# ictnlp/StreamSpeech

Measured on AMD Instinct MI355X. Metric: real-time factor (RTFx = audio seconds / wall seconds) + utterances/sec, offline S2ST fr-en, higher is better.
Workload: dtype f32

## Files before the change

### include/streamspeech_hip.h

```cpp
#ifndef STREAMSPEECH_HIP_H
#define STREAMSPEECH_HIP_H

#include <stddef.h>
#include <stdint.h>

#ifdef __cplusplus
extern "C" {
#endif

#define SS_ABI_VERSION 2

typedef struct ss_model ss_model;
typedef struct ss_vocoder ss_vocoder;
typedef struct ss_scratch ss_scratch;
typedef struct ss_stream_pool ss_stream_pool;

typedef struct ss_config {
  int32_t input_feat, conv_channels, conv_kernel;
  int32_t enc_dim, enc_ffn, enc_heads, enc_layers, dw_kernel;
  int32_t src_vocab, tgt_vocab;
  int32_t mt_layers, dec_dim, dec_ffn, dec_heads;
  int32_t t2u_layers, unit_layers, unit_vocab, ctc_upsample;
  int32_t pad, eos, unk;
  int32_t max_rel_pos;
// ... 418 lines not shown
int ss_debug_last_logits(ss_model* m, void* stream, float* d_out, int64_t cap_floats, int* h_rows, int* h_cols);

int ss_op_ffn_fused(void* stream, const float* dX, int ldx, float* dY, int ldy, const float* ln_g, const float* ln_b,
                    const float* dW1, const float* db1, const float* dW2, const float* db2, float alpha,
                    const float* ln2_g, const float* ln2_b, int M, int D, int F);
int ss_debug_ffn(int grid, int row_tiles_per_wave, int enable);
int ss_debug_rtlin(int grid, int enable);
int ss_debug_conv_c64(int enable);
int ss_debug_conv_c256_rows(int rows);
int ss_debug_conv_c32(int enable);
int ss_debug_conv_c16(int enable);
int64_t ss_debug_enc_step_launches(void);
int ss_op_ln_linear(void* stream, const float* dX, int ldx, const float* ln_g, const float* ln_b, const float* dW,
                    const float* dbias, const float* dR, int ldr, float* dC, int ldc, int M, int N, int K, int act, float alpha,
                    int glu);
int ss_op_ln_linear_ex(void* stream, const float* dX, int ldx, const float* ln_g, const float* ln_b, float* ln_out, const float* dW,
                       const float* dbias, const float* dR, int ldr, float* dC, int ldc, int M, int N, int K, int act, float alpha,
                       int glu, int canon);

int ss_debug_force_tile(int bm, int bn, int ks);
int ss_debug_sk_errors(void);
int ss_debug_attention_split(int v);
int ss_debug_attention_q16(int v);
int ss_debug_enc_step_inject_timeout(ss_model* m);
int ss_debug_scratch_audit(ss_scratch* sc, size_t* booked, size_t* held);
int ss_debug_mt_inject_timeout(ss_model* m);

int ss_op_conv_gemm(void* stream, const float* dA, int lda, const float* dW, const float* dbias,
                    const float* dR, int ldr, const float* dR2, int ldr2, float* dC, int ldc,
                    int M, int N, int Cin, int taps, int dil, int stride, int pad, int in_len,
                    int chunk, int in_act, float in_slope, int act, float alpha, float div, int glu);
typedef struct ss_op_conv_args {
  const float* A; const float* W; const float* bias; const float* R; const float* R2; float* C; float* C2;
  int32_t lda, ldc, ldr, ldr2, ldc2;
  int32_t M, N, Cin, taps, dil, stride, pad, in_len, chunk;
  int32_t in_act; float in_slope;
  int32_t act; float act_slope, alpha, div, c2_slope;
  int32_t glu;
  const int32_t* segs; int32_t nseg, max_seg_out;
  int32_t same_rows;
} ss_op_conv_args;
int ss_op_conv_gemm_ex(void* stream, const ss_op_conv_args* a);
int ss_op_conv_gemm_rows(void* stream, const ss_op_conv_args* a, int m_begin, const int32_t* seg_mb, const float* const* seg_A, int canon);
int ss_op_conv_pair(void* stream, const float* dA, int lda, const float* dW1, const float* db1, const float* dW2, const float* db2,
                    float* dC, int ldc, const float* dR2, int ldr2, float div, float* dC2, int ldc2, float c2_slope, int C, int taps,
                    int dil, int M, int in_len, float slope, const int32_t* d_segs, int nseg);
// ... 123 lines not shown
```

### streamspeech_amd/csrc/attention.hip

```cpp
#include "attn_tile.hpp"

#include <algorithm>
#include <cstdlib>

namespace ss {

void attention_debug_no_mfma(int v) { dispatch_edit([v](Dispatch& d) { d.attn_no_mfma = v; }); }
void attention_debug_q16(int v) { dispatch_edit([v](Dispatch& d) { d.attn_q16 = v; }); }
void attention_debug_split(int v) { dispatch_edit([v](Dispatch& d) { d.attn_split = v; }); }

constexpr int QB = 16;
constexpr int LDKS = DH + 1;

__device__ __forceinline__ float rdlane(float v, int l) {
  return __int_as_float(__builtin_amdgcn_readlane(__float_as_int(v), l));
}

template <bool RELPOS>
__global__ __launch_bounds__(256) void attention_kernel(AttnArgs p) {
  if (p.nseg > 0 && !seg_rebase(p, QB, RELPOS)) return;
  __shared__ float Ks[KT * LDKS];
  __shared__ float Vs[KT * DH];
  __shared__ float Ps[RELPOS ? (KT + QB - 1) * LDKS : 1];

  const int t = threadIdx.x, lane = t & 63, wave = t >> 6;
  const int h = blockIdx.y;
  const int i0 = blockIdx.x * QB;
  const int hoff = h * DH;
  const int qoff = p.Tk - p.Tq;
  const int q0 = p.q0;

  float qu[4], qv[4];
// ... 157 lines not shown
    const float corr = (m_run > -INFINITY) ? expf(m_run - mn) : 0.f;
    l_run = l_run * corr + wave_sum(pe);
    acc *= corr;
    m_run = mn;
#pragma unroll
    for (int u = 0; u < 64; ++u) acc = fmaf(rdlane(pe, u), vv[u], acc);
  }
  if (lane == 0) { part_m[wave] = m_run; part_l[wave] = l_run; }
  part_acc[wave][lane] = acc;
  __syncthreads();
  if (wave == 0) {
    float mt = fmaxf(fmaxf(part_m[0], part_m[1]), fmaxf(part_m[2], part_m[3]));
    float l = 0.f, o = 0.f;
#pragma unroll
    for (int w = 0; w < 4; ++w) {
      const float f = (part_m[w] > -INFINITY) ? expf(part_m[w] - mt) : 0.f;
      l += part_l[w] * f;
      o += part_acc[w][lane] * f;
    }
    p.O[(size_t)i * p.ldo + hoff + lane] = o / l;
  }
}

__global__ __launch_bounds__(256) void attention_mfma_kernel(AttnArgs p) {
  if (p.nseg > 0 && !seg_rebase(p, MQ, false)) return;
  __shared__ __attribute__((aligned(16))) float Ks[KT * LDT];
  __shared__ __attribute__((aligned(16))) float Vt[DH * LDT];
  const int t = threadIdx.x, lane = t & 63, wave = t >> 6;
  const int r = lane & 15, g = lane >> 4;
  const int h = blockIdx.y, hoff = h * DH;
  const int i0 = blockIdx.x * MQ;
  const int qoff = p.Tk - p.Tq;
  const int iq = i0 + wave * 16 + r;
  const bool q_ok = iq < p.Tq;

  f32x4 qf[4];
#pragma unroll
  for (int kk = 0; kk < 4; ++kk) {
    qf[kk] = f32x4{0.f, 0.f, 0.f, 0.f};
    if (q_ok) qf[kk] = *reinterpret_cast<const f32x4*>(p.Q + (size_t)iq * p.ldq + hoff + 16 * kk + 4 * g);
  }
  f32x4 o[4];
#pragma unroll
  for (int dt = 0; dt < 4; ++dt) o[dt] = f32x4{0.f, 0.f, 0.f, 0.f};
  float m_run = -INFINITY, l_run = 0.f;

  int kmax = p.Tk - p.k_mask_tail;
  const int ilast = min(i0 + MQ, p.Tq) - 1;
  if (p.causal) kmax = min(kmax, ilast + qoff + 1);
  if (p.chunk > 0) kmax = min(kmax, (ilast / p.chunk + 1) * p.chunk);
  int lim = p.Tk - p.k_mask_tail;
  if (p.causal) lim = min(lim, iq + qoff + 1);
  if (p.chunk > 0) lim = min(lim, (iq / p.chunk + 1) * p.chunk);
  if (!q_ok) lim = 0;

  for (int j0 = 0; j0 < kmax; j0 += KT) {
    __syncthreads();
    stage_kv_tile(Ks, Vt, p.K, p.V, p.ldk, p.ldv, p.Tk, j0, hoff, t);
    __syncthreads();

    f32x4 s[4];
#pragma unroll
    for (int kt = 0; kt < 4; ++kt) {
      s[kt] = f32x4{0.f, 0.f, 0.f, 0.f};
#pragma unroll
      for (int kk = 0; kk < 4; ++kk) {
        const f32x4 kf = *reinterpret_cast<const f32x4*>(Ks + (kt * 16 + r) * LDT + 16 * kk + 4 * g);
#pragma unroll
        for (int e = 0; e < 4; ++e) s[kt] = __builtin_amdgcn_mfma_f32_16x16x4f32(kf[e], qf[kk][e], s[kt], 0, 0, 0);
      }
    }
    const float corr = softmax_tile(s, j0, lim, p.scale, g, m_run, l_run);
    pv_tile(o, s, Vt, r, g, corr);
  }
  if (q_ok) store_rows(p.O, p.ldo, iq, hoff, g, o, l_run);
}

constexpr int PWIN = 2 * KT;
constexpr size_t kRelposLds = (size_t)(KT * LDT + DH * LDT + PWIN * LDT + 4 * 16 * LDG) * sizeof(float);

template <bool SPLIT>
__global__ __launch_bounds__(256) void attention_relpos_mfma_kernel(AttnArgs p) {
  if (!SPLIT && p.nseg > 0 && !seg_rebase(p, MQ, true)) return;
  extern __shared__ __attribute__((aligned(16))) float smem_rp[];
  float* Ks = smem_rp;
  float* Vt = Ks + KT * LDT;
  float* Ps = Vt + DH * LDT;
  const int t = threadIdx.x, lane = t & 63, wave = t >> 6;
  float* Gs = Ps + PWIN * LDT + wave * 16 * LDG;
  const int r = lane & 15, g = lane >> 4;
  const int h = blockIdx.y, hoff = h * DH;
  int qt = blockIdx.x, sp = 0;
  if (SPLIT) { const int nqt = gridDim.x / p.ksplit; sp = blockIdx.x / nqt; qt = blockIdx.x - sp * nqt; }
  const int i0 = qt * MQ;
  const int q0 = p.q0;
  const int iq = i0 + wave * 16 + r;
  const bool q_ok = iq < p.Tq;

  f32x4 quf[4], qvf[4];
  load_qu_qv(quf, qvf, p.Q, p.ldq, iq, q_ok, p.bias_u, p.bias_v, hoff, g);
  f32x4 o[4];
#pragma unroll
  for (int dt = 0; dt < 4; ++dt) o[dt] = f32x4{0.f, 0.f, 0.f, 0.f};
  float m_run = -INFINITY, l_run = 0.f;

  const int kmax = chunk_bound(p.Tk, p.chunk, min(i0 + MQ, p.Tq) - 1 + q0);
  const int lim = q_ok ? chunk_bound(p.Tk, p.chunk, iq + q0) : 0;
  int jbeg = 0, jend = kmax, s_eff = 1;
  if (SPLIT) {
    const int span = p.ktiles_per_split * KT;
    s_eff = (kmax + span - 1) / span;
    if (sp >= s_eff) return;
    jbeg = sp * span;
    jend = min(kmax, jbeg + span);
  }

  for (int j0 = jbeg; j0 < jend; j0 += KT) {
    __syncthreads();
    stage_kv_tile(Ks, Vt, p.K, p.V, p.ldk, p.ldv, p.Tk, j0, hoff, t);
    {
      const int pbase = j0 - (q0 + i0 + MQ - 1) + p.Tk - 1;
      for (int f = t; f < PWIN * (DH / 4); f += 256) {
        const int row = f >> 4, c4 = (f & 15) * 4;
        const int pr = pbase + row;
        f32x4 pv = {0.f, 0.f, 0.f, 0.f};
        if (row < PWIN - 1 && pr >= 0 && pr < 2 * p.Tk - 1)
          pv = *reinterpret_cast<const f32x4*>(p.P + (size_t)pr * p.ldp + hoff + c4);
        *reinterpret_cast<f32x4*>(Ps + row * LDT + c4) = pv;
      }
    }
    __syncthreads();

    f32x4 s[4];
#pragma unroll
    for (int kt = 0; kt < 4; ++kt) {
      s[kt] = f32x4{0.f, 0.f, 0.f, 0.f};
      f32x4 ga = {0.f, 0.f, 0.f, 0.f}, gb = {0.f, 0.f, 0.f, 0.f};
      const int lrow0 = 16 * (kt - wave) + (MQ - 16);
#pragma unroll
      for (int kk = 0; kk < 4; ++kk) {
        const f32x4 kf = *reinterpret_cast<const f32x4*>(Ks + (kt * 16 + r) * LDT + 16 * kk + 4 * g);
        const f32x4 pa = *reinterpret_cast<const f32x4*>(Ps + (lrow0 + r) * LDT + 16 * kk + 4 * g);
        const f32x4 pb = *reinterpret_cast<const f32x4*>(Ps + (lrow0 + 16 + r) * LDT + 16 * kk + 4 * g);
#pragma unroll
        for (int e = 0; e < 4; ++e) {
          s[kt] = __builtin_amdgcn_mfma_f32_16x16x4f32(kf[e], quf[kk][e], s[kt], 0, 0, 0);
          ga = __builtin_amdgcn_mfma_f32_16x16x4f32(pa[e], qvf[kk][e], ga, 0, 0, 0);
          gb = __builtin_amdgcn_mfma_f32_16x16x4f32(pb[e], qvf[kk][e], gb, 0, 0, 0);
        }
      }
      s[kt] += bd_skew(Gs, r, g, ga, gb);
    }
    const float corr = softmax_tile(s, j0, lim, p.scale, g, m_run, l_run);
    pv_tile(o, s, Vt, r, g, corr);
  }
  if (SPLIT && s_eff > 1) {
    using u32x4 = __attribute__((ext_vector_type(4))) unsigned;
    const int slot0 = (qt * (int)gridDim.y + h) * p.ksplit;
    {
      const __amdgpu_buffer_rsrc_t rs = __builtin_amdgcn_make_buffer_rsrc(
          (void*)(p.part + (size_t)(slot0 + sp) * ATTN_PART_FLOATS), 0, ATTN_PART_FLOATS * 4, 0x00020000);
#pragma unroll
      for (int dt = 0; dt < 4; ++dt) {
        u32x4 v;
#pragma unroll
        for (int e = 0; e < 4; ++e) v[e] = __float_as_uint(o[dt][e]);
        __builtin_amdgcn_raw_buffer_store_b128(v, rs, (dt * 256 + t) * 16, 0, 16);
      }
      const u32x4 ml = {__float_as_uint(m_run), __float_as_uint(l_run), 0u, 0u};
      __builtin_amdgcn_raw_buffer_store_b128(ml, rs, (4 * 256 + t) * 16, 0, 16);
    }
    __shared__ int s_last;
    unsigned* cnt = p.cnt + qt * (int)gridDim.y + h;
    if (!split_arrive(cnt, s_eff, &s_last)) return;
    float mx = -INFINITY;
    for (int g2 = 0; g2 < s_eff; ++g2) {
      const __amdgpu_buffer_rsrc_t rs = __builtin_amdgcn_make_buffer_rsrc(
// ... 168 lines not shown
  SS_LAUNCH_CHECK();
  return SS_OK;
}

int launch_attention(const AttnArgs& a, hipStream_t stream) {
  const int tq = a.nseg > 0 ? a.max_q : a.Tq;
  if (tq <= 0 || (a.nseg == 0 && a.Tk <= 0)) return SS_OK;
  if ((a.ldk & 3) || (a.ldv & 3)) return SS_ERR_ARG;
  const int gz = a.nseg > 0 ? a.nseg : 1;
  if (a.q0 != 0 && (a.nseg > 0 || a.causal)) return SS_ERR_ARG;
  if (a.seg_tail && (a.nseg <= 0 || a.P)) return SS_ERR_ARG;
  if (a.anc) {
    if (a.nseg <= 0 || a.P || tq > 8 || a.q0 != 0 || a.no_decode_kernel || a.anc_ld <= 0 || a.anc_slots <= 0) return SS_ERR_ARG;
    hipLaunchKernelGGL(attention_decode_kernel<true>, dim3(tq, a.H, gz), dim3(256), 0, stream, a);
    SS_LAUNCH_CHECK();
    return SS_OK;
  }
  if (!a.P && tq <= 8 && a.q0 == 0 && !a.no_decode_kernel) {
    hipLaunchKernelGGL(attention_decode_kernel<false>, dim3(tq, a.H, gz), dim3(256), 0, stream, a);
    SS_LAUNCH_CHECK();
    return SS_OK;
  }
  if (!a.P && a.q0 == 0 && !disp().attn_no_mfma && ((a.ldq | a.ldo) & 3) == 0) {
    hipLaunchKernelGGL(attention_mfma_kernel, dim3(cdiv(tq, MQ), a.H, gz), dim3(256), 0, stream, a);
    SS_LAUNCH_CHECK();
    return SS_OK;
  }
  dim3 grid(cdiv(tq, QB), a.H, gz);
  if (a.P) {
    if ((a.nseg == 0 && a.q0 + a.Tq != a.Tk) || (a.ldp & 3) || !a.bias_u || !a.bias_v) return SS_ERR_ARG;
    if (a.nseg > 0 && a.p_tmax <= 0) return SS_ERR_ARG;
    if (!disp().attn_no_mfma && ((a.ldq | a.ldo) & 3) == 0 && a.k_mask_tail == 0 && !a.causal) {
      const int nqt = cdiv(tq, MQ), nkt = cdiv(a.Tk, KT);
      if (a.nseg == 0 && tq <= 48 && disp().attn_q16 && (nkt == 1 || (a.part && cdiv(tq, 16) * a.H <= a.cnt_slots && cdiv(tq, 16) * a.H * nkt <= a.part_slots))) {
        AttnArgs b = a;
        b.ksplit = nkt; b.ktiles_per_split = 1;
        hipLaunchKernelGGL(attention_relpos_q16_kernel, dim3(cdiv(tq, 16) * nkt, a.H, 1), dim3(256), 0, stream, b);
        SS_LAUNCH_CHECK();
        return SS_OK;
      }
      if (a.nseg == 0 && a.part && disp().attn_split >= 0 && nkt >= 2 && nqt * a.H <= a.cnt_slots && nqt * a.H < 128) {
        int tps = disp().attn_split > 0 ? disp().attn_split : cdiv(nkt, std::min(16, std::max(1, 256 / (nqt * a.H))));
        tps = std::max(tps, cdiv(nkt, 16));
        const int S = cdiv(nkt, tps);
        if (S >= 2 && nqt * a.H * S <= a.part_slots) {
          AttnArgs b = a;
          b.ksplit = S; b.ktiles_per_split = tps;
          SS_MAX_LDS_ONCE(&attention_relpos_mfma_kernel<true>, kRelposLds);
          hipLaunchKernelGGL(attention_relpos_mfma_kernel<true>, dim3(nqt * S, a.H, 1), dim3(256), kRelposLds, stream, b);
          SS_LAUNCH_CHECK();
          return SS_OK;
        }
      }
      SS_MAX_LDS_ONCE(&attention_relpos_mfma_kernel<false>, kRelposLds);
      hipLaunchKernelGGL(attention_relpos_mfma_kernel<false>, dim3(nqt, a.H, gz), dim3(256), kRelposLds, stream, a);
      SS_LAUNCH_CHECK();
      return SS_OK;
    }
    hipLaunchKernelGGL(attention_kernel<true>, grid, dim3(256), 0, stream, a);
  } else {
    hipLaunchKernelGGL(attention_kernel<false>, grid, dim3(256), 0, stream, a);
  }
  SS_LAUNCH_CHECK();
  return SS_OK;
}

}
```

### streamspeech_amd/csrc/attention.hpp

```cpp
#pragma once
#include "common.hpp"
#include "dispatch.hpp"

namespace ss {

struct AttnArgs {
  const float* Q = nullptr; const float* K = nullptr; const float* V = nullptr; float* O = nullptr;
  int ldq = 0, ldk = 0, ldv = 0, ldo = 0;
  int Tq = 0, Tk = 0, H = 0;
  float scale = 1.0f;
  int causal = 0;
  int chunk = 0;
  int q0 = 0;
  int k_mask_tail = 0;
  const float* P = nullptr; int ldp = 0;
  const float* bias_u = nullptr; const float* bias_v = nullptr;
  const int* segs = nullptr; int nseg = 0; int max_q = 0; int p_tmax = 0;
  const int* seg_tail = nullptr;
  float* part = nullptr;
  unsigned* cnt = nullptr;
  int part_slots = 0, cnt_slots = 0;
  int ksplit = 0, ktiles_per_split = 0;
  int no_decode_kernel = 0;
  const int* anc = nullptr; int anc_ld = 0; int anc_slots = 0;
};
constexpr int ATTN_PART_FLOATS = 5 * 256 * 4;
constexpr int ATTN_PART_SLOTS = 512, ATTN_CNT_SLOTS = 512;
inline size_t attention_split_bytes() { return (size_t)ATTN_PART_SLOTS * ATTN_PART_FLOATS * sizeof(float) + ATTN_CNT_SLOTS * sizeof(unsigned); }
inline void attention_bind_split(AttnArgs& a, void* scratch) {
  a.part = static_cast<float*>(scratch);
  a.cnt = reinterpret_cast<unsigned*>(a.part + (size_t)ATTN_PART_SLOTS * ATTN_PART_FLOATS);
  a.part_slots = ATTN_PART_SLOTS; a.cnt_slots = ATTN_CNT_SLOTS;
}
void attention_debug_q16(int v);
void attention_debug_split(int v);

int launch_attention(const AttnArgs& a, hipStream_t stream);

struct PoolAttnArgs {
  const float* Qs = nullptr; float* cache = nullptr; float* O = nullptr;
  int ld = 0, ldo = 0, slot_rows = 0;
  const float* P = nullptr; int ldp = 0, p_tmax = 0;
  const float* bias_u = nullptr; const float* bias_v = nullptr;
  const int* sess = nullptr; const int* qt_pre = nullptr;
  int nsess = 0, qtiles = 0, H = 0;
  float scale = 1.f;
};
int launch_attention_pool(const PoolAttnArgs& a, hipStream_t stream);
void attention_debug_no_mfma(int v);

}
```

### streamspeech_amd/csrc/attn_tile.hpp

```cpp
#pragma once
#include "attention.hpp"

namespace ss {

constexpr int KT = 64;
constexpr int DH = 64;
constexpr int MQ = 64;
constexpr int LDT = 68;
constexpr int LDG = 36;
constexpr int Q16_LDO = 68;

using f32x4 = __attribute__((ext_vector_type(4))) float;

__device__ __forceinline__ bool seg_rebase(AttnArgs& p, int rows_per_wg, bool relpos) {
  const int* sg = p.segs + 4 * blockIdx.z;
  p.Tq = sg[1]; p.Tk = sg[3];
  if (p.seg_tail) p.k_mask_tail = p.seg_tail[blockIdx.z];
  if ((int)blockIdx.x * rows_per_wg >= p.Tq) return false;
  p.Q += (size_t)sg[0] * p.ldq; p.O += (size_t)sg[0] * p.ldo;
  p.K += (size_t)sg[2] * p.ldk; p.V += (size_t)sg[2] * p.ldv;
  if (relpos) p.P += (size_t)(p.p_tmax - p.Tk) * p.ldp;
  return true;
}

__device__ __forceinline__ int chunk_bound(int Tk, int chunk, int pos) { return chunk > 0 ? min(Tk, (pos / chunk + 1) * chunk) : Tk; }

__device__ __forceinline__ void stage_kv_tile(float* Ks, float* Vt, const float* K, const float* V, int ldk, int ldv, int Tk, int j0,
                                              int hoff, int t) {
  for (int f = t; f < KT * (DH / 4); f += 256) {
    const int row = f >> 4, c4 = (f & 15) * 4;
    const int j = j0 + row;
    f32x4 kv = {0.f, 0.f, 0.f, 0.f}, vv = kv;
    if (j < Tk) {
      kv = *reinterpret_cast<const f32x4*>(K + (size_t)j * ldk + hoff + c4);
      vv = *reinterpret_cast<const f32x4*>(V + (size_t)j * ldv + hoff + c4);
    }
    *reinterpret_cast<f32x4*>(Ks + row * LDT + c4) = kv;
#pragma unroll
    for (int c = 0; c < 4; ++c) Vt[(c4 + c) * LDT + row] = vv[c];
  }
}

__device__ __forceinline__ float softmax_tile(f32x4 (&s)[4], int j0, int lim, float scale, int g, float& m_run, float& l_run) {
  float mt = -INFINITY;
#pragma unroll
  for (int kt = 0; kt < 4; ++kt)
#pragma unroll
    for (int e = 0; e < 4; ++e) {
      const int j = j0 + kt * 16 + 4 * g + e;
      s[kt][e] = (j < lim) ? s[kt][e] * scale : -INFINITY;
      mt = fmaxf(mt, s[kt][e]);
    }
  mt = fmaxf(mt, __shfl_xor(mt, 16, 64));
  mt = fmaxf(mt, __shfl_xor(mt, 32, 64));
  const float mn = fmaxf(m_run, mt);
  float corr = 1.f, ls = 0.f;
  if (mn > -INFINITY) {
    corr = (m_run > -INFINITY) ? expf(m_run - mn) : 0.f;
#pragma unroll
    for (int kt = 0; kt < 4; ++kt)
#pragma unroll
      for (int e = 0; e < 4; ++e) {
        const float pe = (s[kt][e] > -INFINITY) ? expf(s[kt][e] - mn) : 0.f;
        s[kt][e] = pe;
        ls += pe;
      }
  } else {
#pragma unroll
    for (int kt = 0; kt < 4; ++kt) s[kt] = f32x4{0.f, 0.f, 0.f, 0.f};
  }
  ls += __shfl_xor(ls, 16, 64);
  ls += __shfl_xor(ls, 32, 64);
  l_run = l_run * corr + ls;
  m_run = mn;
  return corr;
}

__device__ __forceinline__ void pv_tile(f32x4 (&o)[4], const f32x4 (&s)[4], const float* Vt, int r, int g, float corr) {
  f32x4 ot[4];
#pragma unroll
  for (int dt = 0; dt < 4; ++dt) ot[dt] = f32x4{0.f, 0.f, 0.f, 0.f};
#pragma unroll
  for (int kt = 0; kt < 4; ++kt)
#pragma unroll
    for (int dt = 0; dt < 4; ++dt) {
      const f32x4 vf = *reinterpret_cast<const f32x4*>(Vt + (dt * 16 + r) * LDT + kt * 16 + 4 * g);
#pragma unroll
      for (int e = 0; e < 4; ++e) ot[dt] = __builtin_amdgcn_mfma_f32_16x16x4f32(vf[e], s[kt][e], ot[dt], 0, 0, 0);
    }
#pragma unroll
  for (int dt = 0; dt < 4; ++dt)
#pragma unroll
    for (int e = 0; e < 4; ++e) o[dt][e] = o[dt][e] * corr + ot[dt][e];
}

__device__ __forceinline__ void store_rows(float* O, int ldo, int iq, int hoff, int g, const f32x4 (&o)[4], float l_run) {
  const float inv = 1.0f / l_run;
#pragma unroll
  for (int dt = 0; dt < 4; ++dt) {
    f32x4 v = o[dt];
#pragma unroll
    for (int e = 0; e < 4; ++e) v[e] *= inv;
    *reinterpret_cast<f32x4*>(O + (size_t)iq * ldo + hoff + 16 * dt + 4 * g) = v;
  }
}

__device__ __forceinline__ void load_qu_qv(f32x4 (&quf)[4], f32x4 (&qvf)[4], const float* Q, int ldq, int iq, bool q_ok,
                                           const float* bias_u, const float* bias_v, int hoff, int g) {
#pragma unroll
  for (int kk = 0; kk < 4; ++kk) {
    const int c = hoff + 16 * kk + 4 * g;
    f32x4 q = {0.f, 0.f, 0.f, 0.f};
// ... 113 lines not shown
```

### streamspeech_amd/csrc/debug_ops.hip

```cpp
#include "model_internal.hpp"
#include "ctc_align.hpp"

static int op_bind_wino(GemmArgs& a, void* stream) {
  static thread_local std::map<hipStream_t, DevBuf> wino_tmps;
  DevBuf& wino_tmp = wino_tmps[(hipStream_t)stream];
  const int N = a.N, Cin = a.Cin, taps = a.taps;
  if ((conv_c64w_enabled() && N == 64 && Cin == 64 && taps >= 3 && conv_c64_eligible(a)) ||
      (conv_c128w_enabled() && N == 128 && Cin == 128 && taps >= 3 && a.same_rows && !a.glu) ||
      (conv_c256w_enabled() && N == 256 && Cin == 256 && taps >= 3 && a.same_rows && !a.glu) ||
      (conv_c32w_enabled() && N == 32 && Cin == 32 && taps >= 3 && conv_c32_eligible(a))) {
    RET(wino_tmp.ensure((size_t)N * ((taps + 2) / 3) * 4 * N * sizeof(float)));
    RET(launch_wino_pack(a.W, wino_tmp.f(), N, taps, (hipStream_t)stream));
    a.Wwino = wino_tmp.f();
  }
  return SS_OK;
}

extern "C" int ss_op_conv_gemm(void* stream, const float* dA, int lda, const float* dW, const float* dbias,
                               const float* dR, int ldr, const float* dR2, int ldr2, float* dC, int ldc, int M,
                               int N, int Cin, int taps, int dil, int stride, int pad, int in_len, int chunk,
                               int in_act, float in_slope, int act, float alpha, float div, int glu) {
  GemmArgs a;
  a.A = dA; a.lda = lda; a.W = dW; a.bias = dbias; a.R = dR; a.ldr = ldr; a.R2 = dR2; a.ldr2 = ldr2; a.C = dC; a.ldc = ldc;
  a.M = M; a.N = N; a.Cin = Cin; a.taps = taps; a.dil = dil; a.stride = stride; a.pad = pad; a.in_len = in_len;
// ... 265 lines not shown
  if (!x) return SS_ERR_ARG;
  AttnProbsArgs a;
  a.Q = x->Q; a.K = x->K; a.ldq = x->ldq; a.ldk = x->ldk; a.H = x->H; a.scale = x->scale;
  a.segs = x->segs; a.nseg = x->nseg; a.q_first = x->q_first; a.row_off = x->row_off;
  a.p_off = reinterpret_cast<const long long*>(x->p_off);
  a.P = x->P; a.peak = x->peak; a.stat = x->stat; a.max_rows = x->max_rows;
  return launch_attention_probs(a, (hipStream_t)stream);
}

extern "C" int ss_op_attention_pool(void* stream, const ss_op_pool_attn_args* x) {
  if (!x) return SS_ERR_ARG;
  PoolAttnArgs a;
  a.Qs = x->Qs; a.cache = x->cache; a.O = x->O;
  a.ld = x->ld; a.ldo = x->ldo; a.slot_rows = x->slot_rows;
  a.P = x->P; a.ldp = x->ldp; a.p_tmax = x->p_tmax;
  a.bias_u = x->bias_u; a.bias_v = x->bias_v;
  a.sess = x->sess; a.qt_pre = x->qt_pre;
  a.nsess = x->nsess; a.qtiles = x->qtiles; a.H = x->H; a.scale = x->scale;
  return launch_attention_pool(a, (hipStream_t)stream);
}

extern "C" int ss_debug_attention_split(int v) { attention_debug_split(v); return SS_OK; }
extern "C" int ss_debug_attention_q16(int v) { attention_debug_q16(v); return SS_OK; }
extern "C" int ss_debug_attention_no_mfma(int v) { attention_debug_no_mfma(v); return SS_OK; }

extern "C" int ss_op_dwconv_bn_silu(void* stream, const float* dx, int ldx, float* dy, int ldy, const float* dwt,
                                    int K, const float* mean, const float* var, const float* gamma,
                                    const float* beta, float eps, int T, int C, int chunk) {
  return launch_dwconv_bn_silu(dx, ldx, dy, ldy, dwt, K, mean, var, gamma, beta, eps, T, C, chunk, (hipStream_t)stream);
}

extern "C" int ss_op_dwconv_bn_silu_ex(void* stream, const float* dx, int ldx, float* dy, int ldy, const float* dwt, int K,
                                       const float* mean, const float* var, const float* gamma, const float* beta, float eps, int T,
                                       int C, int chunk, const int32_t* segs, int nseg, int t_begin) {
  return launch_dwconv_bn_silu(dx, ldx, dy, ldy, dwt, K, mean, var, gamma, beta, eps, T, C, chunk, (hipStream_t)stream, segs, nseg,
                               t_begin);
}

extern "C" int ss_prof_enable(int cls_mask) { prof_enable(cls_mask); return SS_OK; }
extern "C" int ss_prof_enable_hi(int cls_mask) { prof_enable_hi(cls_mask); return SS_OK; }
extern "C" int ss_prof_reset(void) { prof_reset(); return SS_OK; }
extern "C" int ss_prof_read(int cls, double* ms, double* flops, int64_t* launches, double* bytes) {
  long long n = 0;
  int rc = prof_read(cls, ms, flops, &n, bytes);
  if (launches) *launches = n;
  return rc;
// ... 23 lines not shown
```

### streamspeech_amd/csrc/dispatch.hip

```cpp
#include "gemm.hpp"

#include <atomic>
#include <cstdlib>
#include <map>
#include <mutex>
#include <utility>
#include <vector>

namespace ss {

namespace {
std::mutex g_disp_mu;
std::atomic<unsigned> g_disp_gen{1};
Dispatch env_defaults() {
  Dispatch d;
  auto I = [](const char* k, int dflt) { const char* e = getenv(k); return e ? atoi(e) : dflt; };
  auto L = [](const char* k, long long dflt) { const char* e = getenv(k); return e ? atoll(e) : dflt; };
  d.attn_split = I("SS_ATTN_NO_SPLIT", 0) ? -1 : 0; d.attn_q16 = I("SS_ATTN_Q16", d.attn_q16);
  d.c16_off = I("SS_NO_CONV_C16", 0) ? 1 : 0; d.c32_off = I("SS_NO_CONV_C32", 0) ? 1 : 0; d.c64_off = I("SS_NO_CONV_C64", 0) ? 1 : 0;
  d.c16_min_rows = L("SS_CONV_C16_MIN_ROWS", d.c16_min_rows); d.c32_min_rows = L("SS_CONV_C32_MIN_ROWS", d.c32_min_rows);
  d.c64_min_rows = L("SS_CONV_C64_MIN_ROWS", d.c64_min_rows);
  d.c64w_on = I("SS_CONV_C64_WINOGRAD", 1); d.c128w_on = I("SS_CONV_C128_WINOGRAD", 1); d.c256w_on = I("SS_CONV_C256_WINOGRAD", 1);
  d.c32w_on = I("SS_CONV_C32_WINOGRAD", 1); d.c64w_min_k = I("SS_CONV_C64_WINOGRAD_MIN_K", 3);
  d.c128w_min_rows = L("SS_CONV_C128_MIN_ROWS", d.c128w_min_rows); d.c256w_min_rows = L("SS_CONV_C256_MIN_ROWS", d.c256w_min_rows);
  if (const int r = I("SS_CONV_C256_ROWS", d.c256w_rows); r == 128 || r == 256) d.c256w_rows = r;
  if (getenv("SS_FFN_WM")) { d.ffn_wm = I("SS_FFN_WM", 3); d.ffn_wm_forced = 1; d.ffn_wm_env = d.ffn_wm; }
  d.ffn_fusion = I("SS_NO_FFN_FUSION", 0) ? 0 : 1; d.ffn_min_rows = I("SS_FFN_MIN_ROWS", d.ffn_min_rows);
  if (getenv("SS_SK_MIN_GFLOP")) d.sk_min_flops = 1e9 * atof(getenv("SS_SK_MIN_GFLOP"));
  d.no_resblock_fusion = I("SS_NO_RESBLOCK_FUSION", 0); d.no_pair_fusion = I("SS_NO_PAIR_FUSION", 0);
  d.rt_off = I("SS_NO_RTLIN", 0) ? 1 : 0; d.rt_min_rows = I("SS_RTLIN_MIN_ROWS", d.rt_min_rows); d.rt_min_units = L("SS_RTLIN_MIN_UNITS", d.rt_min_units);
  d.rt_kb_min_units = L("SS_RTLIN_KB_MIN_UNITS", d.rt_kb_min_units); d.rt_kb_uw = I("SS_RTLIN_KB_UW", d.rt_kb_uw); d.rt_kb_xmap = I("SS_RTLIN_KB_XMAP", d.rt_kb_xmap);
  d.smallm_max_rows = I("SS_SMALLM_MAX_ROWS", d.smallm_max_rows); d.sk_min_units = L("SS_SK_MIN_UNITS", d.sk_min_units);
  d.no_sk2 = I("SS_NO_SK2", 0) ? 1 : 0; d.sk2_min_k64 = I("SS_SK2_MINK64", d.sk2_min_k64); d.sk2_spare_cus = I("SS_SK2_SPARE_CUS", 0);
  d.rt_wg_per_cu = I("SS_RTLIN_WG_PER_CU", 0); d.c32_min_k = I("SS_CONV_C32_MIN_K", d.c32_min_k); d.c16_min_k = I("SS_CONV_C16_MIN_K", d.c16_min_k);
  return d;
}
Dispatch& process_settings() { static Dispatch d = env_defaults(); return d; }
thread_local const Dispatch* t_disp = nullptr;
thread_local CtxDispatch t_disp_own;
}
void dispatch_edit(const std::function<void(Dispatch&)>& fn) {
// ... 134 lines not shown
```

### streamspeech_amd/csrc/dispatch.hpp

```cpp
#pragma once
#include <functional>

namespace ss {

struct Dispatch {
  int attn_no_mfma = 0;
  int attn_q16 = 1;
  int attn_split = 0;
  int c16_off = 0, c32_off = 0, c64_off = 0;
  long long c16_min_rows = 131072, c32_min_rows = 65536, c64_min_rows = 32768;
  int c64w_on = 1, c128w_on = 1, c256w_on = 1, c32w_on = 1;
  int c64w_min_k = 3;
  long long c128w_min_rows = 65536, c256w_min_rows = 32768;
  int c256w_rows = 128;
  int c32_min_k = 7, c16_min_k = 11;
  int slab_grid_cap = 0;
  int sk_groups = 0;
  int sk2_spare_cus = 0;
  int ffn_force_g = 0;
  int ffn_wm = 3, ffn_wm_forced = 0;
  int ffn_wm_env = 0;
  int ffn_fusion = 1;
  int ffn_min_rows = 1000;
  int force_bm = 0, force_bn = 0, force_ks = 0;
  double sk_min_flops = 4e9;
  int smallm_max_rows = 192;
  long long sk_min_units = 12 * 512;
  int no_sk2 = 0;
  int sk2_min_k64 = 192;
  int no_resblock_fusion = 0, no_pair_fusion = 0;
  int rt_off = 0, rt_min_rows = 193, rt_force_g = 0;
// ... 23 lines not shown
```

### streamspeech_amd/lib.py

```python
import ctypes as C
import os

_HERE = os.path.dirname(os.path.abspath(__file__))
LIB_PATH = os.environ.get("SS_HIP_LIB") or os.path.join(_HERE, "libstreamspeech_hip.so")


class SSConfig(C.Structure):
    _fields_ = [(n, C.c_int32) for n in (
        "input_feat", "conv_channels", "conv_kernel", "enc_dim", "enc_ffn", "enc_heads", "enc_layers",
        "dw_kernel", "src_vocab", "tgt_vocab", "mt_layers", "dec_dim", "dec_ffn", "dec_heads",
        "t2u_layers", "unit_layers", "unit_vocab", "ctc_upsample", "pad", "eos", "unk",
        "max_rel_pos", "max_tgt_pos")]


class SSVocoderConfig(C.Structure):
    _fields_ = [
        ("num_embeddings", C.c_int32), ("embedding_dim", C.c_int32), ("model_in_dim", C.c_int32),
        ("upsample_initial_channel", C.c_int32),
        ("n_up", C.c_int32), ("upsample_rates", C.c_int32 * 8), ("upsample_kernel_sizes", C.c_int32 * 8),
        ("n_res", C.c_int32), ("resblock_kernel_sizes", C.c_int32 * 4), ("resblock_dilations", (C.c_int32 * 3) * 4),
        ("dur_hidden", C.c_int32), ("dur_kernel", C.c_int32)]


_vp, _i, _f, _i64 = C.c_void_p, C.c_int, C.c_float, C.c_int64
# ... 252 lines not shown
    "ss_prof_read": (_i, [_i, C.POINTER(C.c_double), C.POINTER(C.c_double), C.POINTER(_i64), C.POINTER(C.c_double)]),
    "ss_prof_totals": (_i, [_i, C.POINTER(C.c_double), C.POINTER(C.c_double), C.POINTER(_i64)]),
    "ss_prof_read_issued": (_i, [_i, C.POINTER(C.c_double)]),
    "ss_prof_shape_log": (_i, [_i]),
    "ss_prof_shape_dump": (_i, [C.c_char_p, _i]),
    "ss_prof_num_classes": (_i, []),
    "ss_prof_class_name": (C.c_char_p, [_i]),
    "ss_debug_force_tile": (_i, [_i, _i, _i]),
    "ss_op_ffn_fused": (_i, [_vp, _vp, _i, _vp, _i, _vp, _vp, _vp, _vp, _vp, _vp, _f, _vp, _vp, _i, _i, _i]),
    "ss_debug_ffn": (_i, [_i, _i, _i]),
    "ss_debug_rtlin": (_i, [_i, _i]),
    "ss_debug_conv_c64": (_i, [_i]),
    "ss_debug_conv_c256_rows": (_i, [_i]),
    "ss_debug_conv_c32": (_i, [_i]),
    "ss_debug_conv_c16": (_i, [_i]),
    "ss_debug_enc_step_launches": (_i64, []),
    "ss_debug_scratch_audit": (_i, [_vp, C.POINTER(C.c_size_t), C.POINTER(C.c_size_t)]),
    "ss_op_ln_linear": (_i, [_vp, _vp, _i, _vp, _vp, _vp, _vp, _vp, _i, _vp, _i, _i, _i, _i, _i, _f, _i]),
    "ss_op_ln_linear_ex": (_i, [_vp, _vp, _i, _vp, _vp, _vp, _vp, _vp, _vp, _i, _vp, _i, _i, _i, _i, _i, _f, _i, _i]),
    "ss_debug_last_logits": (_i, [_vp, _vp, _vp, _i64, C.POINTER(_i), C.POINTER(_i)]),
    "ss_debug_sk_errors": (_i, []),
    "ss_debug_attention_split": (_i, [_i]),
    "ss_debug_attention_q16": (_i, [_i]),
    "ss_op_conv_gemm": (_i, [_vp, _vp, _i, _vp, _vp, _vp, _i, _vp, _i, _vp, _i, _i, _i, _i, _i, _i, _i, _i, _i, _i,
                             _i, _f, _i, _f, _f, _i]),
    "ss_op_conv_gemm_ex": (_i, [_vp, C.POINTER(SSOpConvArgs)]),
    "ss_op_conv_gemm_rows": (_i, [_vp, C.POINTER(SSOpConvArgs), _i, _vp, _vp, _i]),
    "ss_op_conv_pair": (_i, [_vp, _vp, _i, _vp, _vp, _vp, _vp, _vp, _i, _vp, _i, _f, _vp, _i, _f, _i, _i, _i, _i, _i, _f, _vp, _i]),
    "ss_op_resblock_fused": (_i, [_vp, _vp, _i, _vp, _vp, _vp, _vp, _vp, _vp, _i, _vp, _i, _f, _i, _i, _i, _f, _vp, _i]),
    "ss_debug_slab": (_i, [_i, C.c_longlong]),
    "ss_op_conv_f16": (_i, [_vp, _vp, _vp, _vp, _vp, _vp, _vp, _vp, _i, _i, _i, _i, _i, _f, _i, _f, _vp, _i]),
    "ss_op_layernorm": (_i, [_vp, _vp, _i, _vp, _i, _vp, _vp, _i, _i, _f]),
    "ss_op_attention": (_i, [_vp, _vp, _i, _vp, _i, _vp, _i, _vp, _i, _i, _i, _i, _f, _i, _i, _vp, _i, _vp, _vp]),
    "ss_op_attention_ex": (_i, [_vp, C.POINTER(SSOpAttnArgs)]),
    "ss_op_attention_probs": (_i, [_vp, C.POINTER(SSOpAttnProbsArgs)]),
    "ss_op_attention_pool": (_i, [_vp, C.POINTER(SSOpPoolAttnArgs)]),
    "ss_debug_attention_no_mfma": (_i, [_i]),
    "ss_op_dwconv_bn_silu": (_i, [_vp, _vp, _i, _vp, _i, _vp, _i, _vp, _vp, _vp, _vp, _f, _i, _i, _i]),
    "ss_op_dwconv_bn_silu_ex": (_i, [_vp, _vp, _i, _vp, _i, _vp, _i, _vp, _vp, _vp, _vp, _f, _i, _i, _i, _vp, _i, _i]),
    "ss_op_pool_dwconv": (_i, [_vp, _vp, _vp, _i, _vp, _vp, _i, _vp, _vp, _vp, _vp, _f, _i, _vp, _i, _i]),
    "ss_op_pool_gather_rows": (_i, [_vp, _vp, _vp, _vp, _i, _i, _vp, _vp, _i, _i]),
    "ss_op_pool_gather_ids": (_i, [_vp, _vp, _vp, _vp, _i, _vp, _vp, _i, _i]),
    "ss_op_pool_stack_rows": (_i, [_vp, _vp, _vp, _i, _vp, _vp, _i, _i]),
    "ss_op_masked_argmax": (_i, [_vp, _vp, _i, _i, _i, _i, _i, _i, _i, _vp, _vp, _i, _i, _vp, _i]),
    "ss_op_ctc_collapse": (_i, [_vp, _vp, _i, _i, _i, _vp, _vp, _vp, _vp, _i]),
    "ss_op_masked_argmax_lprob": (_i, [_vp, _vp, _i, _i, _i, _i, _i, _i, _vp, _vp]),
# ... 67 lines not shown
```

Baseline: 6466.

## Skip dead query waves and masked key subtiles; reuse relpos window across tiles

```diff
diff --git a/include/streamspeech_hip.h b/include/streamspeech_hip.h
--- a/include/streamspeech_hip.h
+++ b/include/streamspeech_hip.h
@@ -464,6 +464,7 @@
 int ss_debug_sk_errors(void);
 int ss_debug_attention_split(int v);
 int ss_debug_attention_q16(int v);
+int ss_debug_attention_ref_tiles(int v);
 int ss_debug_enc_step_inject_timeout(ss_model* m);
 int ss_debug_scratch_audit(ss_scratch* sc, size_t* booked, size_t* held);
 int ss_debug_mt_inject_timeout(ss_model* m);
diff --git a/streamspeech_amd/csrc/attention.hip b/streamspeech_amd/csrc/attention.hip
--- a/streamspeech_amd/csrc/attention.hip
+++ b/streamspeech_amd/csrc/attention.hip
@@ -8,6 +8,7 @@
 void attention_debug_no_mfma(int v) { dispatch_edit([v](Dispatch& d) { d.attn_no_mfma = v; }); }
 void attention_debug_q16(int v) { dispatch_edit([v](Dispatch& d) { d.attn_q16 = v; }); }
 void attention_debug_split(int v) { dispatch_edit([v](Dispatch& d) { d.attn_split = v; }); }
+void attention_debug_ref_tiles(int v) { dispatch_edit([v](Dispatch& d) { d.attn_ref_tiles = v ? 1 : 0; }); }
 
 constexpr int QB = 16;
 constexpr int LDKS = DH + 1;
@@ -211,17 +212,20 @@
   }
 }
 
+template <bool REF>
 __global__ __launch_bounds__(256) void attention_mfma_kernel(AttnArgs p) {
   if (p.nseg > 0 && !seg_rebase(p, MQ, false)) return;
   __shared__ __attribute__((aligned(16))) float Ks[KT * LDT];
   __shared__ __attribute__((aligned(16))) float Vt[DH * LDT];
-  const int t = threadIdx.x, lane = t & 63, wave = t >> 6;
+  const int t = threadIdx.x, lane = t & 63;
+  const int wave = __builtin_amdgcn_readfirstlane(t >> 6);
   const int r = lane & 15, g = lane >> 4;
   const int h = blockIdx.y, hoff = h * DH;
   const int i0 = blockIdx.x * MQ;
   const int qoff = p.Tk - p.Tq;
   const int iq = i0 + wave * 16 + r;
   const bool q_ok = iq < p.Tq;
+  const bool wave_live = REF || wave_has_query(i0, wave, p.Tq);
 
   f32x4 qf[4];
 #pragma unroll
@@ -234,24 +238,36 @@
   for (int dt = 0; dt < 4; ++dt) o[dt] = f32x4{0.f, 0.f, 0.f, 0.f};
   float m_run = -INFINITY, l_run = 0.f;
 
-  int kmax = p.Tk - p.k_mask_tail;
-  const int ilast = min(i0 + MQ, p.Tq) - 1;
-  if (p.causal) kmax = min(kmax, ilast + qoff + 1);
-  if (p.chunk > 0) kmax = min(kmax, (ilast / p.chunk + 1) * p.chunk);
-  int lim = p.Tk - p.k_mask_tail;
-  if (p.causal) lim = min(lim, iq + qoff + 1);
-  if (p.chunk > 0) lim = min(lim, (iq / p.chunk + 1) * p.chunk);
-  if (!q_ok) lim = 0;
+  auto bound = [&](int i) {
+    int b = p.Tk - p.k_mask_tail;
+    if (p.causal) b = min(b, i + qoff + 1);
+    if (p.chunk > 0) b = min(b, (i / p.chunk + 1) * p.chunk);
+    return b;
+  };
+  const int kmax = bound(min(i0 + MQ, p.Tq) - 1);
+  const int wmax = bound(min(i0 + 16 * wave + 16, p.Tq) - 1);
+  const int lim = q_ok ? bound(iq) : 0;
 
   for (int j0 = 0; j0 < kmax; j0 += KT) {
     __syncthreads();
-    stage_kv_tile(Ks, Vt, p.K, p.V, p.ldk, p.ldv, p.Tk, j0, hoff, t);
+    if (REF) {
+      stage_kv_tile(Ks, Vt, p.K, p.V, p.ldk, p.ldv, p.Tk, j0, hoff, t);
+    } else {
+      TileRegs rk, rv;
+      rows_request(rk, p.K, p.ldk, 0, p.Tk, j0, hoff, t);
+      rows_request(rv, p.V, p.ldv, 0, p.Tk, j0, hoff, t);
+      rows_commit(rk, Ks, t);
+      rows_commit_t(rv, Vt, t);
+    }
     __syncthreads();
+    if (!wave_live) continue;
+    const int nlive = REF ? 4 : live_subtiles(wmax, j0);
 
     f32x4 s[4];
 #pragma unroll
     for (int kt = 0; kt < 4; ++kt) {
       s[kt] = f32x4{0.f, 0.f, 0.f, 0.f};
+      if (kt >= nlive) continue;
 #pragma unroll
       for (int kk = 0; kk < 4; ++kk) {
         const f32x4 kf = *reinterpret_cast<const f32x4*>(Ks + (kt * 16 + r) * LDT + 16 * kk + 4 * g);
@@ -260,7 +276,7 @@
       }
     }
     const float corr = softmax_tile(s, j0, lim, p.scale, g, m_run, l_run);
-    pv_tile(o, s, Vt, r, g, corr);
+    pv_tile(o, s, Vt, r, g, corr, nlive);
   }
   if (q_ok) store_rows(p.O, p.ldo, iq, hoff, g, o, l_run);
 }
@@ -268,14 +284,17 @@
 constexpr int PWIN = 2 * KT;
 constexpr size_t kRelposLds = (size_t)(KT * LDT + DH * LDT + PWIN * LDT + 4 * 16 * LDG) * sizeof(float);
 
-template <bool SPLIT>
+__device__ __forceinline__ const float* win_rows(const float* Ps, int lr0, int n) { return Ps + ((((lr0 >> 6) + n) & 1) * KT + (lr0 & 63)) * LDT; }
+
+template <bool SPLIT, bool REF>
 __global__ __launch_bounds__(256) void attention_relpos_mfma_kernel(AttnArgs p) {
   if (!SPLIT && p.nseg > 0 && !seg_rebase(p, MQ, true)) return;
   extern __shared__ __attribute__((aligned(16))) float smem_rp[];
   float* Ks = smem_rp;
   float* Vt = Ks + KT * LDT;
   float* Ps = Vt + DH * LDT;
-  const int t = threadIdx.x, lane = t & 63, wave = t >> 6;
+  const int t = threadIdx.x, lane = t & 63;
+  const int wave = __builtin_amdgcn_readfirstlane(t >> 6);
   float* Gs = Ps + PWIN * LDT + wave * 16 * LDG;
   const int r = lane & 15, g = lane >> 4;
   const int h = blockIdx.y, hoff = h * DH;
@@ -285,6 +304,7 @@
   const int q0 = p.q0;
   const int iq = i0 + wave * 16 + r;
   const bool q_ok = iq < p.Tq;
+  const bool wave_live = REF || wave_has_query(i0, wave, p.Tq);
 
   f32x4 quf[4], qvf[4];
   load_qu_qv(quf, qvf, p.Q, p.ldq, iq, q_ok, p.bias_u, p.bias_v, hoff, g);
@@ -294,6 +314,7 @@
   float m_run = -INFINITY, l_run = 0.f;
 
   const int kmax = chunk_bound(p.Tk, p.chunk, min(i0 + MQ, p.Tq) - 1 + q0);
+  const int wmax = chunk_bound(p.Tk, p.chunk, min(i0 + 16 * wave + 16, p.Tq) - 1 + q0);
   const int lim = q_ok ? chunk_bound(p.Tk, p.chunk, iq + q0) : 0;
   int jbeg = 0, jend = kmax, s_eff = 1;
   if (SPLIT) {
@@ -304,44 +325,69 @@
     jend = min(kmax, jbeg + span);
   }
 
-  for (int j0 = jbeg; j0 < jend; j0 += KT) {
+  const int pzero = p.Tk - 1 - (q0 + i0 + MQ - 1);
+  const int plim = 2 * p.Tk - 1;
+  if (!REF) {
+    TileRegs rlo;
+    rows_request(rlo, p.P, p.ldp, 0, plim, pzero + jbeg, hoff, t);
+    rows_commit(rlo, Ps, t);
+  }
+  for (int j0 = jbeg, tile = 0; j0 < jend; j0 += KT, ++tile) {
+    const int n = REF ? 0 : tile;
     __syncthreads();
-    stage_kv_tile(Ks, Vt, p.K, p.V, p.ldk, p.ldv, p.Tk, j0, hoff, t);
-    {
-      const int pbase = j0 - (q0 + i0 + MQ - 1) + p.Tk - 1;
+    if (REF) {
+      stage_kv_tile(Ks, Vt, p.K, p.V, p.ldk, p.ldv, p.Tk, j0, hoff, t);
+      const int pbase = pzero + j0;
       for (int f = t; f < PWIN * (DH / 4); f += 256) {
         const int row = f >> 4, c4 = (f & 15) * 4;
         const int pr = pbase + row;
         f32x4 pv = {0.f, 0.f, 0.f, 0.f};
-        if (row < PWIN - 1 && pr >= 0 && pr < 2 * p.Tk - 1)
+        if (row < PWIN - 1 && pr >= 0 && pr < plim)
           pv = *reinterpret_cast<const f32x4*>(p.P + (size_t)pr * p.ldp + hoff + c4);
         *reinterpret_cast<f32x4*>(Ps + row * LDT + c4) = pv;
       }
+    } else {
+      TileRegs rk, rv, rhi;
+      const int pu = pzero + j0 + KT;
+      rows_request(rk, p.K, p.ldk, 0, p.Tk, j0, hoff, t);
+      rows_request(rv, p.V, p.ldv, 0, p.Tk, j0, hoff, t);
+      rows_request(rhi, p.P, p.ldp, 0, j0 + KT < jend ? plim : min(plim, pu + KT - 1), pu, hoff, t);
+      rows_commit(rk, Ks, t);
+      rows_commit_t(rv, Vt, t);
+      rows_commit(rhi, Ps + ((n + 1) & 1) * KT * LDT, t);
     }
     __syncthreads();
-
-    f32x4 s[4];
+    if (!wave_live) continue;
+    const int nlive = REF ? 4 : live_subtiles(wmax, j0);
+
+    auto g_tile = [&](int c) {
+      const float* pw = win_rows(Ps, 16 * (c - wave) + (MQ - 16), n) + r * LDT + 4 * g;
+      f32x4 gt = {0.f, 0.f, 0.f, 0.f};
+#pragma unroll
+      for (int kk = 0; kk < 4; ++kk) {
+        const f32x4 pa = *reinterpret_cast<const f32x4*>(pw + 16 * kk);
+#pragma unroll
+        for (int e = 0; e < 4; ++e) gt = __builtin_amdgcn_mfma_f32_16x16x4f32(pa[e], qvf[kk][e], gt, 0, 0, 0);
+      }
+      return gt;
+    };
+    f32x4 s[4], gnext = {0.f, 0.f, 0.f, 0.f};
 #pragma unroll
     for (int kt = 0; kt < 4; ++kt) {
       s[kt] = f32x4{0.f, 0.f, 0.f, 0.f};
-      f32x4 ga = {0.f, 0.f, 0.f, 0.f}, gb = {0.f, 0.f, 0.f, 0.f};
-      const int lrow0 = 16 * (kt - wave) + (MQ - 16);
+      if (kt >= nlive) continue;
+      const f32x4 ga = (REF || kt == 0) ? g_tile(kt) : gnext;
+      gnext = g_tile(kt + 1);
 #pragma unroll
       for (int kk = 0; kk < 4; ++kk) {
         const f32x4 kf = *reinterpret_cast<const f32x4*>(Ks + (kt * 16 + r) * LDT + 16 * kk + 4 * g);
-        const f32x4 pa = *reinterpret_cast<const f32x4*>(Ps + (lrow0 + r) * LDT + 16 * kk + 4 * g);
-        const f32x4 pb = *reinterpret_cast<const f32x4*>(Ps + (lrow0 + 16 + r) * LDT + 16 * kk + 4 * g);
-#pragma unroll
-        for (int e = 0; e < 4; ++e) {
-          s[kt] = __builtin_amdgcn_mfma_f32_16x16x4f32(kf[e], quf[kk][e], s[kt], 0, 0, 0);
-          ga = __builtin_amdgcn_mfma_f32_16x16x4f32(pa[e], qvf[kk][e], ga, 0, 0, 0);
-          gb = __builtin_amdgcn_mfma_f32_16x16x4f32(pb[e], qvf[kk][e], gb, 0, 0, 0);
-        }
-      }
-      s[kt] += bd_skew(Gs, r, g, ga, gb);
+#pragma unroll
+        for (int e = 0; e < 4; ++e) s[kt] = __builtin_amdgcn_mfma_f32_16x16x4f32(kf[e], quf[kk][e], s[kt], 0, 0, 0);
+      }
+      s[kt] += bd_skew(Gs, r, g, ga, gnext);
     }
     const float corr = softmax_tile(s, j0, lim, p.scale, g, m_run, l_run);
-    pv_tile(o, s, Vt, r, g, corr);
+    pv_tile(o, s, Vt, r, g, corr, nlive);
   }
   if (SPLIT && s_eff > 1) {
     using u32x4 = __attribute__((ext_vector_type(4))) unsigned;
@@ -556,7 +602,8 @@
     return SS_OK;
   }
   if (!a.P && a.q0 == 0 && !disp().attn_no_mfma && ((a.ldq | a.ldo) & 3) == 0) {
-    hipLaunchKernelGGL(attention_mfma_kernel, dim3(cdiv(tq, MQ), a.H, gz), dim3(256), 0, stream, a);
+    if (disp().attn_ref_tiles) hipLaunchKernelGGL(attention_mfma_kernel<true>, dim3(cdiv(tq, MQ), a.H, gz), dim3(256), 0, stream, a);
+    else hipLaunchKernelGGL(attention_mfma_kernel<false>, dim3(cdiv(tq, MQ), a.H, gz), dim3(256), 0, stream, a);
     SS_LAUNCH_CHECK();
     return SS_OK;
   }
@@ -580,14 +627,24 @@
         if (S >= 2 && nqt * a.H * S <= a.part_slots) {
           AttnArgs b = a;
           b.ksplit = S; b.ktiles_per_split = tps;
-          SS_MAX_LDS_ONCE(&attention_relpos_mfma_kernel<true>, kRelposLds);
-          hipLaunchKernelGGL(attention_relpos_mfma_kernel<true>, dim3(nqt * S, a.H, 1), dim3(256), kRelposLds, stream, b);
+          if (disp().attn_ref_tiles) {
+            SS_MAX_LDS_ONCE((&attention_relpos_mfma_kernel<true, true>), kRelposLds);
+            hipLaunchKernelGGL((attention_relpos_mfma_kernel<true, true>), dim3(nqt * S, a.H, 1), dim3(256), kRelposLds, stream, b);
+          } else {
+            SS_MAX_LDS_ONCE((&attention_relpos_mfma_kernel<true, false>), kRelposLds);
+            hipLaunchKernelGGL((attention_relpos_mfma_kernel<true, false>), dim3(nqt * S, a.H, 1), dim3(256), kRelposLds, stream, b);
+          }
           SS_LAUNCH_CHECK();
           return SS_OK;
         }
       }
-      SS_MAX_LDS_ONCE(&attention_relpos_mfma_kernel<false>, kRelposLds);
-      hipLaunchKernelGGL(attention_relpos_mfma_kernel<false>, dim3(nqt, a.H, gz), dim3(256), kRelposLds, stream, a);
+      if (disp().attn_ref_tiles) {
+        SS_MAX_LDS_ONCE((&attention_relpos_mfma_kernel<false, true>), kRelposLds);
+        hipLaunchKernelGGL((attention_relpos_mfma_kernel<false, true>), dim3(nqt, a.H, gz), dim3(256), kRelposLds, stream, a);
+      } else {
+        SS_MAX_LDS_ONCE((&attention_relpos_mfma_kernel<false, false>), kRelposLds);
+        hipLaunchKernelGGL((attention_relpos_mfma_kernel<false, false>), dim3(nqt, a.H, gz), dim3(256), kRelposLds, stream, a);
+      }
       SS_LAUNCH_CHECK();
       return SS_OK;
     }
diff --git a/streamspeech_amd/csrc/attention.hpp b/streamspeech_amd/csrc/attention.hpp
--- a/streamspeech_amd/csrc/attention.hpp
+++ b/streamspeech_amd/csrc/attention.hpp
@@ -34,6 +34,7 @@
 }
 void attention_debug_q16(int v);
 void attention_debug_split(int v);
+void attention_debug_ref_tiles(int v);
 
 int launch_attention(const AttnArgs& a, hipStream_t stream);
 
diff --git a/streamspeech_amd/csrc/attn_tile.hpp b/streamspeech_amd/csrc/attn_tile.hpp
--- a/streamspeech_amd/csrc/attn_tile.hpp
+++ b/streamspeech_amd/csrc/attn_tile.hpp
@@ -25,6 +25,26 @@
 
 __device__ __forceinline__ int chunk_bound(int Tk, int chunk, int pos) { return chunk > 0 ? min(Tk, (pos / chunk + 1) * chunk) : Tk; }
 
+struct TileRegs { f32x4 x[4]; };
+__device__ __forceinline__ void rows_request(TileRegs& a, const float* src, int ld, int jlo, int jhi, int j0, int hoff, int t) {
+#pragma unroll
+  for (int i = 0; i < 4; ++i) {
+    const int j = j0 + (t >> 4) + 16 * i;
+    a.x[i] = f32x4{0.f, 0.f, 0.f, 0.f};
+    if (j >= jlo && j < jhi) a.x[i] = *reinterpret_cast<const f32x4*>(src + (size_t)j * ld + hoff + (t & 15) * 4);
+  }
+}
+__device__ __forceinline__ void rows_commit(const TileRegs& a, float* dst, int t) {
+#pragma unroll
+  for (int i = 0; i < 4; ++i) *reinterpret_cast<f32x4*>(dst + ((t >> 4) + 16 * i) * LDT + (t & 15) * 4) = a.x[i];
+}
+__device__ __forceinline__ void rows_commit_t(const TileRegs& a, float* dst, int t) {
+#pragma unroll
+  for (int i = 0; i < 4; ++i)
+#pragma unroll
+    for (int c = 0; c < 4; ++c) dst[((t & 15) * 4 + c) * LDT + (t >> 4) + 16 * i] = a.x[i][c];
+}
+
 __device__ __forceinline__ void stage_kv_tile(float* Ks, float* Vt, const float* K, const float* V, int ldk, int ldv, int Tk, int j0,
                                               int hoff, int t) {
   for (int f = t; f < KT * (DH / 4); f += 256) {
@@ -41,6 +61,9 @@
   }
 }
 
+__device__ __forceinline__ bool wave_has_query(int i0, int wave, int Tq) { return __builtin_amdgcn_readfirstlane(i0 + 16 * wave < Tq ? 1 : 0) != 0; }
+__device__ __forceinline__ int live_subtiles(int wmax, int j0) { return __builtin_amdgcn_readfirstlane(max(0, min(4, (wmax - j0 + 15) >> 4))); }
+
 __device__ __forceinline__ float softmax_tile(f32x4 (&s)[4], int j0, int lim, float scale, int g, float& m_run, float& l_run) {
   float mt = -INFINITY;
 #pragma unroll
@@ -76,18 +99,20 @@
   return corr;
 }
 
-__device__ __forceinline__ void pv_tile(f32x4 (&o)[4], const f32x4 (&s)[4], const float* Vt, int r, int g, float corr) {
+__device__ __forceinline__ void pv_tile(f32x4 (&o)[4], const f32x4 (&s)[4], const float* Vt, int r, int g, float corr, int nlive) {
   f32x4 ot[4];
 #pragma unroll
   for (int dt = 0; dt < 4; ++dt) ot[dt] = f32x4{0.f, 0.f, 0.f, 0.f};
 #pragma unroll
-  for (int kt = 0; kt < 4; ++kt)
+  for (int kt = 0; kt < 4; ++kt) {
+    if (kt >= nlive) break;
 #pragma unroll
     for (int dt = 0; dt < 4; ++dt) {
       const f32x4 vf = *reinterpret_cast<const f32x4*>(Vt + (dt * 16 + r) * LDT + kt * 16 + 4 * g);
 #pragma unroll
       for (int e = 0; e < 4; ++e) ot[dt] = __builtin_amdgcn_mfma_f32_16x16x4f32(vf[e], s[kt][e], ot[dt], 0, 0, 0);
     }
+  }
 #pragma unroll
   for (int dt = 0; dt < 4; ++dt)
 #pragma unroll
diff --git a/streamspeech_amd/csrc/debug_ops.hip b/streamspeech_amd/csrc/debug_ops.hip
--- a/streamspeech_amd/csrc/debug_ops.hip
+++ b/streamspeech_amd/csrc/debug_ops.hip
@@ -311,6 +311,7 @@
 
 extern "C" int ss_debug_attention_split(int v) { attention_debug_split(v); return SS_OK; }
 extern "C" int ss_debug_attention_q16(int v) { attention_debug_q16(v); return SS_OK; }
+extern "C" int ss_debug_attention_ref_tiles(int v) { attention_debug_ref_tiles(v); return SS_OK; }
 extern "C" int ss_debug_attention_no_mfma(int v) { attention_debug_no_mfma(v); return SS_OK; }
 
 extern "C" int ss_op_dwconv_bn_silu(void* stream, const float* dx, int ldx, float* dy, int ldy, const float* dwt,
diff --git a/streamspeech_amd/csrc/dispatch.hip b/streamspeech_amd/csrc/dispatch.hip
--- a/streamspeech_amd/csrc/dispatch.hip
+++ b/streamspeech_amd/csrc/dispatch.hip
@@ -17,6 +17,7 @@
   auto I = [](const char* k, int dflt) { const char* e = getenv(k); return e ? atoi(e) : dflt; };
   auto L = [](const char* k, long long dflt) { const char* e = getenv(k); return e ? atoll(e) : dflt; };
   d.attn_split = I("SS_ATTN_NO_SPLIT", 0) ? -1 : 0; d.attn_q16 = I("SS_ATTN_Q16", d.attn_q16);
+  d.attn_ref_tiles = I("SS_ATTN_REF_TILES", 0) ? 1 : 0;
   d.c16_off = I("SS_NO_CONV_C16", 0) ? 1 : 0; d.c32_off = I("SS_NO_CONV_C32", 0) ? 1 : 0; d.c64_off = I("SS_NO_CONV_C64", 0) ? 1 : 0;
   d.c16_min_rows = L("SS_CONV_C16_MIN_ROWS", d.c16_min_rows); d.c32_min_rows = L("SS_CONV_C32_MIN_ROWS", d.c32_min_rows);
   d.c64_min_rows = L("SS_CONV_C64_MIN_ROWS", d.c64_min_rows);
diff --git a/streamspeech_amd/csrc/dispatch.hpp b/streamspeech_amd/csrc/dispatch.hpp
--- a/streamspeech_amd/csrc/dispatch.hpp
+++ b/streamspeech_amd/csrc/dispatch.hpp
@@ -7,6 +7,7 @@
   int attn_no_mfma = 0;
   int attn_q16 = 1;
   int attn_split = 0;
+  int attn_ref_tiles = 0;
   int c16_off = 0, c32_off = 0, c64_off = 0;
   long long c16_min_rows = 131072, c32_min_rows = 65536, c64_min_rows = 32768;
   int c64w_on = 1, c128w_on = 1, c256w_on = 1, c32w_on = 1;
diff --git a/streamspeech_amd/lib.py b/streamspeech_amd/lib.py
--- a/streamspeech_amd/lib.py
+++ b/streamspeech_amd/lib.py
@@ -298,6 +298,7 @@
     "ss_debug_sk_errors": (_i, []),
     "ss_debug_attention_split": (_i, [_i]),
     "ss_debug_attention_q16": (_i, [_i]),
+    "ss_debug_attention_ref_tiles": (_i, [_i]),
     "ss_op_conv_gemm": (_i, [_vp, _vp, _i, _vp, _vp, _vp, _i, _vp, _i, _vp, _i, _i, _i, _i, _i, _i, _i, _i, _i, _i,
                              _i, _f, _i, _f, _f, _i]),
     "ss_op_conv_gemm_ex": (_i, [_vp, C.POINTER(SSOpConvArgs)]),
```

New measurement: 6493 (median of 6 runs). Within noise of the previous version (+0.4%).
